# zilliztech/knowhere

Measured on NVIDIA H100. Metric: queries/sec at recall@10>=0.95, 10Mx128 f32 IVF_PQ, higher is better.
Workload: dtype f32

## Files before the change

### knowhere_b200/csrc/kb2_ivfpq_tc.cuh

```cuda
#pragma once
#include <cuda_bf16.h>

#include <type_traits>
#include <utility>

#include "kb2_gemm_tc.cuh"
#include "kb2_ivf.cuh"
#include "kb2_listmajor.cuh"

namespace kb2 {
namespace pqtc {

using lm::TM;
constexpr int NQT = 256;
constexpr int THREADS = 512;
constexpr int GROUP_THREADS = 128;
constexpr int MAXW = 80;
constexpr int META_BYTES = 3 * NQT * 4;
template <int G, int DSUB>
struct TcCfg {
    static constexpr int M = 16 * G;
    static constexpr int KD = M * DSUB;
    static_assert(KD % 16 == 0 && (DSUB == 2 || DSUB == 4 || DSUB == 8), "unsupported PQ geometry");
    static constexpr int XCHUNK = KD / 8;
    static constexpr int KSTEPS = KD / 16 + 1;
    static constexpr int CHUNKS = 2 * KSTEPS;
    static constexpr int GRP_BYTES = CHUNKS * 128;
    static constexpr int TAB_BYTES = M * 256 * DSUB * 2;
    static constexpr int A_BYTES = (TM / 8) * GRP_BYTES, B_BYTES = (NQT / 8) * GRP_BYTES;
    static constexpr int OFF_TAB = 0;
    static constexpr int OFF_A = TAB_BYTES;
    static constexpr int OFF_B = OFF_A + 2 * A_BYTES;
    static constexpr int OFF_META = OFF_B + B_BYTES;
    static constexpr int OFF_BAR = OFF_META + 2 * META_BYTES;
    static constexpr size_t SMEM_BYTES = OFF_BAR + 256 + 128 ;
    static_assert(SMEM_BYTES <= 227 * 1024, "filter kernel shared memory");
};
constexpr int KD = 128;
constexpr float kErrCoef = 0.0085f;
constexpr float kAccCoef = 4e-5f;

struct Params {
    int metric;
    int nq, nprobe;
    const float* queries;
    const __nv_bfloat16* qb16;
    const float* qnorm;
    const int32_t* n_items;
    int32_t* ticket;
    const int32_t* item_list;
    const int32_t* item_q0;
    const int32_t* item_nq;
    const int32_t* pair_q;
    const float* pair_base;
    const float* bound;
    int k_need;
    float margin_coef;
    float rmax;
    const int64_t* list_off;
    const int32_t* list_len;
    const uint4* codes;
    const uint4* codes_plain;
    int64_t npad;
    const float* t1;
    const float* pqc;
    const uint4* pqc16;
    const uint8_t* bitset;
    const int32_t* rows;
    uint4* log;
    uint32_t* log_cnt;
    uint32_t log_cap;
    uint32_t* qflag;
    unsigned long long* counters;
};

template <typename F, int... I>
__device__ __forceinline__ void
static_for_impl(F&& f, std::integer_sequence<int, I...>) {
    (f(std::integral_constant<int, I>{}), ...);
}
template <int N, typename F>
__device__ __forceinline__ void
static_for(F&& f) {
    static_for_impl(f, std::make_integer_sequence<int, N>{});
}
template <int C0_, int W_>
struct BlockCols {
    static constexpr int C0 = C0_, W = W_;
};
template <int LO, int HI, typename F>
__device__ __forceinline__ void
dispatch_range(int n, F&& f) {
    if constexpr (LO == HI) {
        f(std::integral_constant<int, LO>{});
    } else {
        constexpr int MID = (LO + HI) / 2;
        if (n <= MID) dispatch_range<LO, MID>(n, f);
        else dispatch_range<MID + 1, HI>(n, f);
    }
}

__device__ __forceinline__ void
bar_sync_epi() {
    asm volatile("bar.sync 1, 256;" ::: "memory");
}
__device__ __forceinline__ uint64_t
make_desc_ns(uint32_t smem_addr, uint32_t grp_bytes) {
    uint64_t d = 0;
    d |= (uint64_t)((smem_addr & 0x3FFFFu) >> 4);
    d |= (uint64_t)(128 >> 4) << 16;
    d |= (uint64_t)(grp_bytes >> 4) << 32;
    return d;
}

#ifdef KB2_FILTER_STALLS
#define KB2_STALL_BEGIN(v) const long long v = clock64()
#define KB2_STALL_END(slot, v) stall[slot] += clock64() - (v)
constexpr int kStallMaxCtas = 1024, kStallSlots = 8;
__device__ unsigned long long g_filter_stalls[kStallMaxCtas][2][2][kStallSlots];
__global__ void
filter_stalls_print_kernel(int ctas) {
    for (int b = 0; b < min(ctas, kStallMaxCtas); b++) {
        printf("KB2STALL cta=%d", b);
        for (int r = 0; r < 2; r++) {
            printf(r == 0 ? " dec=" : " cons=");
            for (int i = 0; i < kStallSlots; i++)
                printf(i ? ",%llu" : "%llu", g_filter_stalls[b][r][0][i] + g_filter_stalls[b][r][1][i]);
        }
        printf("\n");
    }
}
#else
#define KB2_STALL_BEGIN(v)
#define KB2_STALL_END(slot, v)
#endif

__device__ __forceinline__ void
split3_bf16(float x, uint32_t& hi, uint32_t& mid, uint32_t& lo) {
    const __nv_bfloat16 h = __float2bfloat16_rn(x);
    hi = (uint32_t)__bfloat16_as_ushort(h);
    if (!(fabsf(x) < INFINITY)) { mid = 0u; lo = 0u; return; }
    const float r1 = x - __bfloat162float(h);
    const __nv_bfloat16 m = __float2bfloat16_rn(r1);
    const float r2 = r1 - __bfloat162float(m);
    mid = (uint32_t)__bfloat16_as_ushort(m);
    lo = (uint32_t)__bfloat16_as_ushort(__float2bfloat16_rn(r2));
}

template <int METRIC, int G, int DSUB>
__global__ void __launch_bounds__(THREADS, 1)
ivfpq_tc_filter_kernel(Params p) {
    using C = TcCfg<G, DSUB>;
    constexpr int KD = C::KD, XCHUNK = C::XCHUNK, KSTEPS = C::KSTEPS, GRP_BYTES = C::GRP_BYTES, TAB_BYTES = C::TAB_BYTES;
    constexpr int A_BYTES = C::A_BYTES, OFF_TAB = C::OFF_TAB, OFF_A = C::OFF_A, OFF_B = C::OFF_B, OFF_META = C::OFF_META,
                  OFF_BAR = C::OFF_BAR;
    extern __shared__ unsigned char smem_dyn[];
    const uint32_t raw = tc::smem_u32(smem_dyn);
    const uint32_t base = (raw + 127u) & ~127u;
    unsigned char* sm = smem_dyn + (base - raw);
    const uint32_t bars = base + OFF_BAR;
    auto bar_a_full = [&](int i) { return bars + 8u * i; };
    auto bar_a_empty = [&](int i) { return bars + 8u * (2 + i); };
    const uint32_t bar_b_full = bars + 8u * 8, bar_b_free = bars + 8u * 9;
    auto bar_meta_full = [&](int i) { return bars + 8u * (10 + i); };
    auto bar_meta_free = [&](int i) { return bars + 8u * (12 + i); };
    uint32_t* qcnt = (uint32_t*)(sm + OFF_BAR + 8 * 15);

    const int warp = __shfl_sync(0xffffffffu, (int)threadIdx.x >> 5, 0), lane = threadIdx.x & 31;
    const int n_items = *p.n_items;

    const lm::ItemRing<8> ring(sm + OFF_BAR + 144, p.ticket);
    ring.init();

    if (threadIdx.x == 0) {
        for (int i = 0; i < 2; i++) {
            tc::mbar_init(bar_a_full(i), GROUP_THREADS);
            tc::mbar_init(bar_a_empty(i), GROUP_THREADS);
            tc::mbar_init(bar_meta_full(i), 2 * GROUP_THREADS);
            tc::mbar_init(bar_meta_free(i), 2 * GROUP_THREADS);
        }
        tc::mbar_init(bar_b_full, 2 * GROUP_THREADS);
        tc::mbar_init(bar_b_free, 2 * GROUP_THREADS);
        qcnt[0] = qcnt[1] = qcnt[2] = qcnt[3] = 0;
        asm volatile("fence.mbarrier_init.release.cluster;" ::: "memory");
    }
#ifdef KB2_FILTER_STALLS
    long long stall[kStallSlots] = {0, 0, 0, 0, 0, 0, 0, 0};
    KB2_STALL_BEGIN(t_role);
#endif
    {
        uint4* tab = (uint4*)(sm + OFF_TAB);
        for (int i = threadIdx.x; i < TAB_BYTES / 16; i += THREADS) tab[i] = __ldg(p.pqc16 + i);
    }
    __syncthreads();
    const float inv_alpha = (METRIC == KB2_METRIC_L2) ? 0.5f : 1.f;

    if (warp < 8) {
        const int dt = threadIdx.x;
        const int dg = dt >> 7;
        const int tid = dt & 127;
        const uint4* tab = (const uint4*)(sm + OFF_TAB);
        auto write_meta = [&](int item, int it) {
            KB2_STALL_BEGIN(t_meta);
            const int par = it & 1;
            tc::mbar_wait(bar_meta_free(par), (((uint32_t)it >> 1) & 1u) ^ 1u);
            const int q0 = p.item_q0[item];
            const int nqi = p.item_nq[item];
            float* m_h = (float*)(sm + OFF_META + par * META_BYTES);
            float* m_base = m_h + NQT;
            int* m_q = (int*)(m_base + NQT);
            const int j = dt;
            float h = -INFINITY, bs = 0.f;
            int q = -1;
            if (j < nqi) {
                q = p.pair_q[q0 + j];
                bs = p.pair_base[q0 + j];
                const float bnd = p.bound[q];
                if (!(bnd < INFINITY)) {
                    p.qflag[q] = 1u;
                    if (p.counters) atomicAdd(p.counters + 6, 1ull << 32);
                } else {
                    const float margin = p.margin_coef * p.qnorm[q] * 1.01f + 1e-30f;
                    const float h0 = (bnd + margin - bs) * inv_alpha;
                    h = h0 + kAccCoef * (fabsf(h0) + p.rmax) + 1e-30f;
                }
            }
            m_h[j] = h;
            m_base[j] = bs;
            m_q[j] = q;
            tc::mbar_arrive(bar_meta_full(par));
            KB2_STALL_END(5, t_meta);
        };
        uint32_t g0 = 0;
        int it = 0;
        int item = ring.at_warp(0);
        if (item < n_items) write_meta(item, 0);
        for (; item < n_items; it++) {
            const int item_next = ring.at_warp(it + 1);
            const int l = p.item_list[item];
            const int nqi = p.item_nq[item];
            const int nmma = (nqi + 15) & ~15;
            const int len = p.list_len[l];
            const int64_t off = p.list_off[l];
            const int ntiles = (len + TM - 1) / TM;
            const int par = it & 1;
            const int t_first = (int)((dg - (int)(g0 & 1u)) & 1);
            uint4 w_next[G];
#pragma unroll
            for (int g = 0; g < G; g++) w_next[g] = make_uint4(0, 0, 0, 0);
            float t_next = 0.f;
            const uint4* code_src = (DSUB == 8) ? p.codes : p.codes_plain;
            if (t_first < ntiles && off + (int64_t)t_first * TM + tid < p.npad) {
#pragma unroll
                for (int g = 0; g < G; g++) w_next[g] = ldg_stream_u4(code_src + (int64_t)g * p.npad + off + (int64_t)t_first * TM + tid);
                if (METRIC == KB2_METRIC_L2) t_next = __ldg(p.t1 + off + (int64_t)t_first * TM + tid);
            }
            auto decode_tile = [&](int t) {
                KB2_STALL_BEGIN(t_dec);
                const uint32_t g = g0 + (uint32_t)t;
                uint4 w[G];
#pragma unroll
                for (int gg = 0; gg < G; gg++) w[gg] = w_next[gg];
                const float tv = t_next;
                {
                    const int64_t pn = off + (int64_t)(t + 2) * TM + tid;
                    if (t + 2 < ntiles && pn < p.npad) {
#pragma unroll
                        for (int gg = 0; gg < G; gg++) w_next[gg] = ldg_stream_u4(code_src + (int64_t)gg * p.npad + pn);
                        if (METRIC == KB2_METRIC_L2) t_next = __ldg(p.t1 + pn);
                    }
                }
                float r = INFINITY;
                if (t * TM + tid < len) r = (METRIC == KB2_METRIC_L2) ? 0.5f * tv : 0.f;
                uint32_t rh, rm, rl;
                split3_bf16(-r, rh, rm, rl);
                uint4 v[XCHUNK];
                if constexpr (DSUB == 8) {
#pragma unroll
                    for (int gg = 0; gg < G; gg++) {
                        const uint32_t ww[4] = {w[gg].x, w[gg].y, w[gg].z, w[gg].w};
#pragma unroll
                        for (int s = 0; s < 16; s++) {
                            const uint32_t byte = (ww[s >> 2] >> (8 * (s & 3))) & 255u;
                            v[gg * 16 + s] = tab[byte * (16 * G) + gg * 16 + ((s + tid) & 15)];
                        }
                    }
                } else {
                    constexpr int SPC = 8 / DSUB;
                    constexpr int WPS = DSUB / 2;
                    const uint32_t* tab32 = reinterpret_cast<const uint32_t*>(tab);
#pragma unroll
                    for (int c = 0; c < XCHUNK; c++) {
                        uint32_t u[4];
#pragma unroll
                        for (int j = 0; j < SPC; j++) {
                            const int m = c * SPC + j;
                            const uint4 wg = w[m >> 4];
                            const int b = m & 15;
                            const uint32_t word = (b < 4) ? wg.x : (b < 8) ? wg.y : (b < 12) ? wg.z : wg.w;
                            const uint32_t byte = (word >> (8 * (b & 3))) & 255u;
#pragma unroll
                            for (int x = 0; x < WPS; x++) u[j * WPS + x] = tab32[(m * 256 + byte) * WPS + x];
                        }
                        v[c] = make_uint4(u[0], u[1], u[2], u[3]);
                    }
                }
                KB2_STALL_BEGIN(t_ae);
                tc::mbar_wait(bar_a_empty(dg), ((g >> 1) & 1u) ^ 1u);
                KB2_STALL_END(1, t_ae);
                unsigned char* A = sm + OFF_A + dg * A_BYTES + (tid >> 3) * GRP_BYTES + (tid & 7) * 16;
#pragma unroll
                for (int c = 0; c < XCHUNK; c++) {
                    const int chunk = (DSUB == 8) ? (c & ~15) + ((c + tid) & 15) : c;
                    *reinterpret_cast<uint4*>(A + chunk * 128) = v[c];
                }
                *reinterpret_cast<uint4*>(A + XCHUNK * 128) = make_uint4(rh | (rm << 16), rl | (0x3F80u << 16), 0x3F803F80u, 0u);
                *reinterpret_cast<uint4*>(A + (XCHUNK + 1) * 128) = make_uint4(0u, 0u, 0u, 0u);
                tc::fence_proxy_async();
                tc::mbar_arrive(bar_a_full(dg));
                KB2_STALL_END(3, t_dec);
            };
            if (t_first < ntiles) decode_tile(t_first);
            KB2_STALL_BEGIN(t_b);
            asm volatile("bar.sync 2, 256;" ::: "memory");
            KB2_STALL_BEGIN(t_bf);
            tc::mbar_wait(bar_b_free, ((uint32_t)it & 1u) ^ 1u);
            KB2_STALL_END(2, t_bf);
            {
                const float* m_h = (const float*)(sm + OFF_META + par * META_BYTES);
                const int* m_q = (const int*)(m_h + 2 * NQT);
                const uint32_t Bs = base + OFF_B;
                unsigned char* B = sm + OFF_B;
                const int kc = tid >> 3;
                const int rsub = tid & 7;
                for (int blk = dg; blk < nmma / 8 && kc < XCHUNK; blk += 2) {
                    const int row = blk * 8 + rsub;
                    const int q = m_q[row];
                    const uint32_t dst = (uint32_t)(blk * GRP_BYTES + kc * 128 + rsub * 16);
                    if (q >= 0) {
                        const void* src = reinterpret_cast<const uint4*>(p.qb16 + (int64_t)q * KD) + kc;
                        asm volatile("cp.async.cg.shared.global [%0], [%1], 16;" ::"r"(Bs + dst), "l"(src) : "memory");
                    } else {
                        *reinterpret_cast<uint4*>(B + dst) = make_uint4(0, 0, 0, 0);
                    }
                }
                if (dt < nmma) {
                    uint32_t hh, hm, hl;
                    split3_bf16(m_h[dt], hh, hm, hl);
                    unsigned char* Bc = B + (dt >> 3) * GRP_BYTES + (dt & 7) * 16;
                    *reinterpret_cast<uint4*>(Bc + XCHUNK * 128) = make_uint4(0x3F803F80u, 0x3F80u | (hh << 16), hm | (hl << 16), 0u);
                    *reinterpret_cast<uint4*>(Bc + (XCHUNK + 1) * 128) = make_uint4(0u, 0u, 0u, 0u);
                }
                asm volatile("cp.async.wait_all;" ::: "memory");
            }
            tc::fence_proxy_async();
            tc::mbar_arrive(bar_b_full);
            KB2_STALL_END(4, t_b);
            if (item_next < n_items) write_meta(item_next, it + 1);
            for (int t = t_first + 2; t < ntiles; t += 2) decode_tile(t);
            g0 += (uint32_t)ntiles;
            item = item_next;
        }
    } else {
        const int et = threadIdx.x - 256;
        const int eg = et >> 7;
        const int e = et & 127;
        const int we = warp & 3;
        const uint32_t n_logs = 2u * gridDim.x;
        uint4* my_log = p.log + (size_t)(2 * blockIdx.x + eg) * p.log_cap;
        uint32_t* my_cursor = qcnt + eg;
        bool log_over = false;
        unsigned long long n_codes = 0;
        uint32_t g0 = 0;
        int it = 0;
        for (int item = ring.at_warp(0); item < n_items; item = ring.at_warp(++it)) {
            const int l = p.item_list[item];
            const int nqi = p.item_nq[item];
            const int ncls = __shfl_sync(0xffffffffu, (nqi + 15) >> 4, 0);
            const int len = p.list_len[l];
            const int64_t off = p.list_off[l];
            const int ntiles = (len + TM - 1) / TM;
            const int par = it & 1;
            KB2_STALL_BEGIN(t_mf);
            tc::mbar_wait(bar_meta_full(par), ((uint32_t)it >> 1) & 1u);
            KB2_STALL_END(1, t_mf);
            const float* m_base = (const float*)(sm + OFF_META + par * META_BYTES) + NQT;
            const int* m_q = (const int*)(m_base + NQT);
            if (et == 0) n_codes += (unsigned long long)len * (unsigned long long)nqi;
            const int t_first = (int)((eg - (int)(g0 & 1u)) & 1);
            KB2_STALL_BEGIN(t_bfull);
            tc::mbar_wait(bar_b_full, (uint32_t)it & 1u);
            KB2_STALL_END(2, t_bfull);
            const uint32_t a0 = base + OFF_A + eg * A_BYTES;
            const uint32_t b0 = base + OFF_B;
            const uint32_t la0 = (uint32_t)make_desc_ns(a0, GRP_BYTES), lb0 = (uint32_t)make_desc_ns(b0, GRP_BYTES);
            constexpr uint64_t desc_hi = (uint64_t)(GRP_BYTES >> 4) << 32;
            for (int t = t_first; t < ntiles; t += 2) {
                const uint32_t g = g0 + (uint32_t)t;
                KB2_STALL_BEGIN(t_af);
                tc::mbar_wait(bar_a_full(eg), (g >> 1) & 1u);
                KB2_STALL_END(3, t_af);
                auto issue = [&](auto& acc, int h, auto blk) {
                    using B = decltype(blk);
                    KB2_STALL_BEGIN(t_is);
                    uint32_t la = la0 + (uint32_t)(h * 8 * GRP_BYTES / 16), lb = lb0 + (uint32_t)(B::C0 / 8 * GRP_BYTES / 16);
                    if constexpr (G == 1) asm volatile("" : "+r"(la), "+r"(lb));
                    tc::fence_operand(acc);
                    tc::wgmma_fence();
#pragma unroll
                    for (int ks = 0; ks < KSTEPS; ks++)
                        tc::wgmma_bf16<B::W>(acc, desc_hi | (la + ks * 16u), desc_hi | (lb + ks * 16u), ks > 0 ? 1u : 0u);
                    tc::wgmma_commit();
                    tc::fence_operand(acc);
                    KB2_STALL_END(6, t_is);
                };
                uint64_t mh[2][2] = {{0ull, 0ull}, {0ull, 0ull}};
                auto test = [&](const auto& v, int h, auto blk) {
                    using B = decltype(blk);
                    constexpr int NBIT = B::W / 4, HALF = NBIT / 2;
                    KB2_STALL_BEGIN(t_te);
                    uint32_t n0l = 0u, n0h = 0u, n1l = 0u, n1h = 0u;
#pragma unroll
                    for (int i = HALF - 1; i >= 0; i--) {
                        const int x = 4 * (i >> 1) + (i & 1);
                        const int xh = 4 * ((i + HALF) >> 1) + ((i + HALF) & 1);
                        n0l = __funnelshift_l(__float_as_uint(v[x]), n0l, 1);
                        n0h = __funnelshift_l(__float_as_uint(v[xh]), n0h, 1);
                        n1l = __funnelshift_l(__float_as_uint(v[x + 2]), n1l, 1);
                        n1h = __funnelshift_l(__float_as_uint(v[xh + 2]), n1h, 1);
                    }
                    constexpr uint32_t mask = (1u << NBIT) - 1u;
                    const uint32_t m0 = ~((n0h << HALF) | n0l) & mask, m1 = ~((n1h << HALF) | n1l) & mask;
                    mh[h][0] |= (uint64_t)m0 << (B::C0 / 4);
                    mh[h][1] |= (uint64_t)m1 << (B::C0 / 4);
                    KB2_STALL_END(7, t_te);
                };
                auto flush = [&]() {
                    const uint32_t total =
                        (uint32_t)(__popcll(mh[0][0]) + __popcll(mh[0][1]) + __popcll(mh[1][0]) + __popcll(mh[1][1]));
                    if (total != 0u) {
                        uint32_t slot = atomicAdd(my_cursor, total);
#pragma unroll
                        for (int h = 0; h < 2; h++) {
#pragma unroll
                            for (int i = 0; i < 2; i++) {
                                const int rel = t * TM + h * 64 + we * 16 + (lane >> 2) + 8 * i;
                                uint64_t m = mh[h][i];
                                while (m) {
                                    const int bit = __ffsll((long long)m) - 1;
                                    m &= m - 1;
                                    const int col = 8 * (bit >> 1) + 2 * (lane & 3) + (bit & 1);
                                    if (slot < p.log_cap) {
                                        uint4 o;
                                        o.x = (uint32_t)m_q[col];
                                        o.y = (uint32_t)(off + rel);
                                        o.z = __float_as_uint(m_base[col]);
                                        o.w = 0u;
                                        my_log[slot] = o;
                                    } else {
                                        log_over = true;
                                    }
                                    slot++;
                                }
                            }
                        }
                    }
                };
                dispatch_range<1, NQT / 16>(ncls, [&](auto nc) {
                    constexpr int NC = decltype(nc)::value, NB = (16 * NC + MAXW - 1) / MAXW, NBT = 2 * NB;
                    constexpr int U = NC / NB, X = NC % NB;
                    auto blk = [](auto cc) {
                        constexpr int c = decltype(cc)::value;
                        return BlockCols<16 * (c * U + (c < X ? c : X)), 16 * (U + (c < X ? 1 : 0))>{};
                    };
                    float va[8 * (U + (X > 0 ? 1 : 0))], vb[8 * (U + (X > 0 ? 1 : 0))];
                    issue(va, 0, blk(std::integral_constant<int, 0>{}));
                    static_for<NBT>([&](auto bc) {
                        constexpr int b = decltype(bc)::value;
                        if constexpr (b + 1 < NBT) {
                            constexpr auto bn = blk(std::integral_constant<int, (b + 1) % NB>{});
                            if constexpr ((b + 1) & 1) issue(vb, (b + 1) / NB, bn);
                            else issue(va, (b + 1) / NB, bn);
                            KB2_STALL_BEGIN(t_w);
                            tc::wgmma_wait<1>();
                            KB2_STALL_END(4, t_w);
                        } else {
                            KB2_STALL_BEGIN(t_w);
                            tc::wgmma_wait<0>();
                            KB2_STALL_END(4, t_w);
                        }
                        constexpr auto bb = blk(std::integral_constant<int, b % NB>{});
                        if constexpr (b & 1) {
                            tc::fence_operand(vb);
                            test(vb, b / NB, bb);
                        } else {
                            tc::fence_operand(va);
                            test(va, b / NB, bb);
                        }
                    });
                });
                tc::mbar_arrive(bar_a_empty(eg));
                KB2_STALL_BEGIN(t_fl);
                flush();
                KB2_STALL_END(5, t_fl);
            }
            tc::mbar_arrive(bar_b_free);
            tc::mbar_arrive(bar_meta_free(par));
            g0 += (uint32_t)ntiles;
        }
        if (log_over) p.log_cnt[n_logs] = 1u;
        if (eg == 0) asm volatile("bar.sync 3, 128;" ::: "memory"); else asm volatile("bar.sync 4, 128;" ::: "memory");
        if (e == 0) {
            const uint32_t n = min(*my_cursor, p.log_cap);
            p.log_cnt[2 * blockIdx.x + eg] = n;
            if (p.counters) atomicAdd(p.counters + 2, (unsigned long long)n);
        }
        if (et == 0 && p.counters) atomicAdd(p.counters, n_codes);
    }
#ifdef KB2_FILTER_STALLS
    KB2_STALL_END(0, t_role);
    if ((threadIdx.x & 127) == 0 && blockIdx.x < kStallMaxCtas) {
        for (int i = 0; i < kStallSlots; i++)
            g_filter_stalls[blockIdx.x][warp >= 8][(threadIdx.x >> 7) & 1][i] = (unsigned long long)stall[i];
    }
#endif
}

__global__ void
prepare_queries_kernel(const float* __restrict__ q, int64_t nq, int d, __nv_bfloat16* __restrict__ qb16, float* __restrict__ qnorm) {
    const int64_t w = ((int64_t)blockIdx.x * blockDim.x + threadIdx.x) >> 5;
    const int lane = threadIdx.x & 31;
    if (w >= nq) return;
    float s = 0.f;
    for (int j = lane * 4; j < d; j += 128) {
        const float4 v = __ldg(reinterpret_cast<const float4*>(q + w * d + j));
        __nv_bfloat162 lo = __floats2bfloat162_rn(v.x, v.y), hi = __floats2bfloat162_rn(v.z, v.w);
        uint2 o;
        o.x = *reinterpret_cast<uint32_t*>(&lo);
        o.y = *reinterpret_cast<uint32_t*>(&hi);
        *reinterpret_cast<uint2*>(qb16 + w * d + j) = o;
        s += v.x * v.x + v.y * v.y + v.z * v.z + v.w * v.w;
    }
    s = warp_sum(s);
    if (lane == 0) qnorm[w] = sqrtf(s) * 1.0001f;
}

__global__ void __launch_bounds__(256)
prepare_tables_kernel(const float* __restrict__ pqc, int dsub, __nv_bfloat16* __restrict__ pqc16, float* __restrict__ maxn2) {
    const int m = blockIdx.x, j = threadIdx.x;
    const int M = gridDim.x;
    const float* c = pqc + ((size_t)m * 256 + j) * dsub;
    float n2 = 0.f;
    __nv_bfloat16* o = pqc16 + (dsub == 8 ? ((size_t)j * M + m) : ((size_t)m * 256 + j)) * dsub;
    for (int t = 0; t < dsub; t++) {
        n2 = fmaf(c[t], c[t], n2);
        o[t] = __float2bfloat16_rn(c[t]);
    }
    __shared__ float red[256];
    red[j] = n2;
    __syncthreads();
    for (int s = 128; s > 0; s >>= 1) {
        if (j < s) red[j] = fmaxf(red[j], red[j + s]);
        __syncthreads();
    }
    if (j == 0) maxn2[m] = red[0];
}
__global__ void
unrotate_codes_kernel(const uint8_t* __restrict__ rot, int64_t total_words , int64_t npad, uint8_t* __restrict__ plain) {
    const int64_t t = (int64_t)blockIdx.x * blockDim.x + threadIdx.x;
    if (t >= total_words * 16) return;
    const int s = (int)(t & 15);
    const int64_t word = t >> 4;
    const int64_t pos = word % npad;
    plain[word * 16 + ((s + (int)(pos & 15)) & 15)] = rot[t];
}

template <int METRIC>
__global__ void __launch_bounds__(256, 1)
lut_build_kernel(const float* __restrict__ queries, int64_t nq, const int32_t* __restrict__ qlist, const uint32_t* __restrict__ qcount,
                 const float* __restrict__ pqc, float* __restrict__ lut) {
    __shared__ __align__(16) float s_q[2][KD];
    const int j = threadIdx.x;
    const float scale = (METRIC == KB2_METRIC_L2) ? -2.f : -1.f;
    if (qlist) nq = (int64_t)*qcount;
    float4 c[32];
#pragma unroll
    for (int m = 0; m < 16; m++) {
        const float* cp = pqc + ((size_t)m * 256 + j) * 8;
        c[2 * m] = __ldg(reinterpret_cast<const float4*>(cp));
        c[2 * m + 1] = __ldg(reinterpret_cast<const float4*>(cp + 4));
    }
    const int64_t per = (nq + gridDim.x - 1) / gridDim.x;
    const int64_t q_beg = (int64_t)blockIdx.x * per, q_end = min(nq, q_beg + per);
    auto qrow = [&](int64_t i) { return queries + (qlist ? (int64_t)qlist[i] : i) * KD; };
    if (q_beg < q_end && threadIdx.x < KD) s_q[0][threadIdx.x] = qrow(q_beg)[threadIdx.x];
    __syncthreads();
    for (int64_t q = q_beg; q < q_end; q++) {
        const int cur = (int)((q - q_beg) & 1);
        if (q + 1 < q_end && threadIdx.x < KD) s_q[cur ^ 1][threadIdx.x] = qrow(q + 1)[threadIdx.x];
        float* dst = lut + q * 4096 + j * 16;
#pragma unroll
        for (int m4 = 0; m4 < 16; m4 += 4) {
            float o[4];
#pragma unroll
            for (int u = 0; u < 4; u++) {
                const int m = m4 + u;
                const float4 qa = *reinterpret_cast<const float4*>(&s_q[cur][m * 8]);
                const float4 qb = *reinterpret_cast<const float4*>(&s_q[cur][m * 8 + 4]);
                float a = 0.f;
                a = fmaf(qa.x, c[2 * m].x, a); a = fmaf(qa.y, c[2 * m].y, a); a = fmaf(qa.z, c[2 * m].z, a); a = fmaf(qa.w, c[2 * m].w, a);
                a = fmaf(qb.x, c[2 * m + 1].x, a); a = fmaf(qb.y, c[2 * m + 1].y, a); a = fmaf(qb.z, c[2 * m + 1].z, a); a = fmaf(qb.w, c[2 * m + 1].w, a);
                o[u] = a * scale;
            }
            *reinterpret_cast<float4*>(dst + m4) = make_float4(o[0], o[1], o[2], o[3]);
        }
        __syncthreads();
    }
}

template <int METRIC, int G, int DSUB>
__global__ void __launch_bounds__(128)
exact_eval_kernel(const float* __restrict__ queries, const float* __restrict__ pqc, const float* __restrict__ lut,
                  const float* __restrict__ bound_of,
                  const uint4* __restrict__ codes, int64_t npad, const float* __restrict__ t1, const uint8_t* __restrict__ bitset,
                  const int32_t* __restrict__ rows, uint64_t* __restrict__ cand, uint32_t* __restrict__ cand_cnt, int cap,
                  uint32_t* __restrict__ qflag, const uint32_t* __restrict__ log_over, int k_trim = 0) {
    constexpr int KDIM = 16 * G * DSUB;
    __shared__ __align__(16) float s_q[KDIM];
    __shared__ uint32_t s_h[256];
    __shared__ float s_red[8];
    __shared__ uint32_t s_ctl[2];
    const int64_t q = blockIdx.x;
    if (*log_over) {
        if (threadIdx.x == 0) qflag[q] = 1u;
        return;
    }
    if (qflag[q]) return;
    const uint32_t n = min(cand_cnt[q], (uint32_t)cap);
    if (n == 0) return;
    const bool use_lut = (G == 1 && DSUB == 8) && lut != nullptr;
    if (!use_lut) {
        for (int j = threadIdx.x; j < KDIM; j += 128) s_q[j] = queries[q * KDIM + j];
        __syncthreads();
    }
    const float* lq = lut + q * 4096;
    const float bound = bound_of[q];
    const float scale = (METRIC == KB2_METRIC_L2) ? -2.f : -1.f;
    uint64_t* row = cand + q * cap;
    auto eval = [&](uint64_t ent, float& key_out) -> uint64_t {
        const uint32_t pos = (uint32_t)ent;
        const float base = __uint_as_float((uint32_t)(ent >> 32));
        float acc0 = (METRIC == KB2_METRIC_L2) ? __ldg(t1 + pos) : 0.f, acc1 = 0.f;
#pragma unroll
        for (int g = 0; g < G; g++) {
            const uint4 w = __ldg(codes + (int64_t)g * npad + pos);
            const uint32_t ww[4] = {w.x, w.y, w.z, w.w};
#pragma unroll
            for (int s = 0; s < 16; s++) {
                const uint32_t byte = (ww[s >> 2] >> (8 * (s & 3))) & 255u;
                const uint32_t m = g * 16 + ((pos + s) & 15u);
                float v;
                if (use_lut) {
                    v = __ldg(lq + byte * 16 + m);
                } else {
                    const float* c = pqc + ((size_t)m * 256 + byte) * DSUB;
                    const float* qs = &s_q[m * DSUB];
                    float a = 0.f;
#pragma unroll
                    for (int t = 0; t < DSUB; t++) a = fmaf(qs[t], __ldg(c + t), a);
                    v = __fmul_rn(a, scale);
                }
                if (s & 1) acc1 = __fadd_rn(acc1, v); else acc0 = __fadd_rn(acc0, v);
            }
        }
        const float key = __fadd_rn(base, __fadd_rn(acc0, acc1));
        bool keep = key <= bound;
        if (keep && bitset) keep = !bit_is_set(bitset, rows[pos]);
        key_out = keep ? key : INFINITY;
        return keep ? pack_kp(key, pos) : kEmpty;
    };
    if (k_trim > 0 && n <= 512u && n > (uint32_t)k_trim) {
        uint64_t pk[4];
        float kf[4];
        float lo = INFINITY, hi = -INFINITY;
        s_h[threadIdx.x] = 0;
        s_h[threadIdx.x + 128] = 0;
        if (threadIdx.x == 0) s_ctl[1] = 0;
#pragma unroll
        for (int it = 0; it < 4; it++) {
            const uint32_t i = threadIdx.x + it * 128;
            pk[it] = kEmpty;
            kf[it] = INFINITY;
            if (i < n) pk[it] = eval(row[i], kf[it]);
            if (kf[it] < INFINITY) { lo = fminf(lo, kf[it]); hi = fmaxf(hi, kf[it]); }
        }
#pragma unroll
        for (int o = 16; o > 0; o >>= 1) {
            lo = fminf(lo, __shfl_xor_sync(0xffffffffu, lo, o));
            hi = fmaxf(hi, __shfl_xor_sync(0xffffffffu, hi, o));
        }
        if ((threadIdx.x & 31) == 0) { s_red[threadIdx.x >> 5] = lo; s_red[4 + (threadIdx.x >> 5)] = hi; }
        __syncthreads();
        lo = fminf(fminf(s_red[0], s_red[1]), fminf(s_red[2], s_red[3]));
        hi = fmaxf(fmaxf(s_red[4], s_red[5]), fmaxf(s_red[6], s_red[7]));
        const float sc = (hi > lo) ? 256.f / (hi - lo) : 0.f;
        int bin[4];
#pragma unroll
        for (int it = 0; it < 4; it++) {
            bin[it] = 256;
            if (kf[it] < INFINITY) {
                bin[it] = min(255, (int)((kf[it] - lo) * sc));
                atomicAdd(&s_h[bin[it]], 1u);
            }
        }
        __syncthreads();
        if (threadIdx.x < 32) {
            const int lane = threadIdx.x;
            uint32_t h[8], sum = 0;
#pragma unroll
            for (int t = 0; t < 8; t++) { h[t] = s_h[lane * 8 + t]; sum += h[t]; }
            uint32_t incl = sum;
#pragma unroll
            for (int o = 1; o < 32; o <<= 1) {
                const uint32_t v = __shfl_up_sync(0xffffffffu, incl, o);
                if (lane >= o) incl += v;
            }
            const uint32_t excl = incl - sum;
            const uint32_t total = __shfl_sync(0xffffffffu, incl, 31);
            if (lane == 0 && total < (uint32_t)k_trim) s_ctl[0] = 255u;
            if (excl < (uint32_t)k_trim && incl >= (uint32_t)k_trim) {
                uint32_t run = excl;
                int b = lane * 8 + 7;
#pragma unroll
                for (int t = 0; t < 8; t++) {
                    run += h[t];
                    if (run >= (uint32_t)k_trim) { b = lane * 8 + t; break; }
                }
                s_ctl[0] = (uint32_t)b;
            }
        }
        __syncthreads();
        const int bstar = (int)s_ctl[0];
#pragma unroll
        for (int it = 0; it < 4; it++)
            if (bin[it] <= bstar) row[atomicAdd(&s_ctl[1], 1u)] = pk[it];
        __syncthreads();
        if (threadIdx.x == 0) cand_cnt[q] = s_ctl[1];
        return;
    }
    float lo = INFINITY, hi = -INFINITY;
    for (uint32_t i = threadIdx.x; i < n; i += 128) {
        float kf;
        row[i] = eval(row[i], kf);
        if (kf < INFINITY) { lo = fminf(lo, kf); hi = fmaxf(hi, kf); }
    }
    if (k_trim > 0 && k_trim <= 96 && n > 512u) {
        __shared__ uint64_t s_stage[128];
        s_h[threadIdx.x] = 0;
        s_h[threadIdx.x + 128] = 0;
        if (threadIdx.x == 0) { s_ctl[0] = 0xffffffffu; s_ctl[1] = 0; }
#pragma unroll
        for (int o = 16; o > 0; o >>= 1) {
            lo = fminf(lo, __shfl_xor_sync(0xffffffffu, lo, o));
            hi = fmaxf(hi, __shfl_xor_sync(0xffffffffu, hi, o));
        }
        if ((threadIdx.x & 31) == 0) { s_red[threadIdx.x >> 5] = lo; s_red[4 + (threadIdx.x >> 5)] = hi; }
        __syncthreads();
        lo = fminf(fminf(s_red[0], s_red[1]), fminf(s_red[2], s_red[3]));
        hi = fmaxf(fmaxf(s_red[4], s_red[5]), fmaxf(s_red[6], s_red[7]));
        const float sc = (hi > lo) ? 256.f / (hi - lo) : 0.f;
        for (uint32_t i = threadIdx.x; i < n; i += 128) {
            const uint64_t e = row[i];
            if (e != kEmpty) atomicAdd(&s_h[min(255, (int)((unpack_key(e) - lo) * sc))], 1u);
        }
        __syncthreads();
        if (threadIdx.x < 32) {
            const int lane = threadIdx.x;
            uint32_t h[8], sum = 0;
#pragma unroll
            for (int t = 0; t < 8; t++) { h[t] = s_h[lane * 8 + t]; sum += h[t]; }
            uint32_t incl = sum;
#pragma unroll
            for (int o = 1; o < 32; o <<= 1) {
                const uint32_t v = __shfl_up_sync(0xffffffffu, incl, o);
                if (lane >= o) incl += v;
            }
            const uint32_t excl = incl - sum;
            if (excl < (uint32_t)k_trim && incl >= (uint32_t)k_trim) {
                uint32_t run = excl;
                int b = lane * 8 + 7;
#pragma unroll
                for (int t = 0; t < 8; t++) {
                    run += h[t];
                    if (run >= (uint32_t)k_trim) { b = lane * 8 + t; break; }
                }
                if (run <= 128u) s_ctl[0] = (uint32_t)b;
            }
        }
        __syncthreads();
        const uint32_t bstar = s_ctl[0];
        if (bstar == 0xffffffffu) return;
        for (uint32_t i = threadIdx.x; i < n; i += 128) {
            const uint64_t e = row[i];
            if (e != kEmpty && (uint32_t)min(255, (int)((unpack_key(e) - lo) * sc)) <= bstar) s_stage[atomicAdd(&s_ctl[1], 1u)] = e;
        }
        __syncthreads();
        const uint32_t nk = s_ctl[1];
        for (uint32_t i = threadIdx.x; i < nk; i += 128) row[i] = s_stage[i];
        if (threadIdx.x == 0) cand_cnt[q] = nk;
    }
}

__global__ void __launch_bounds__(1024)
compact_resp_kernel(const int64_t* __restrict__ probe_ids, int nprobe, int64_t nq, const int32_t* __restrict__ list_owner, int rank,
                    int32_t* __restrict__ list, uint32_t* __restrict__ count) {
    __shared__ uint32_t s_n;
    if (threadIdx.x == 0) s_n = 0;
    __syncthreads();
    for (int64_t q = threadIdx.x; q < nq; q += 1024) {
        const int64_t l = probe_ids[q * nprobe];
        if (l >= 0 && list_owner[l] == rank) list[atomicAdd(&s_n, 1u)] = (int32_t)q;
    }
    __syncthreads();
    if (threadIdx.x == 0) *count = s_n;
}
__global__ void
fill_f32_kernel(float* __restrict__ out, int64_t n, float v) {
    const int64_t i = (int64_t)blockIdx.x * blockDim.x + threadIdx.x;
    if (i < n) out[i] = v;
}
__global__ void __launch_bounds__(256)
max_abs_kernel(const float* __restrict__ x, int64_t n, uint32_t* __restrict__ out) {
    float m = 0.f;
    for (int64_t i = (int64_t)blockIdx.x * blockDim.x + threadIdx.x; i < n; i += (int64_t)gridDim.x * blockDim.x) m = fmaxf(m, fabsf(x[i]));
#pragma unroll
    for (int o = 16; o > 0; o >>= 1) m = fmaxf(m, __shfl_xor_sync(0xffffffffu, m, o));
    if ((threadIdx.x & 31) == 0 && m > 0.f) atomicMax(out, __float_as_uint(m));
}

__global__ void __launch_bounds__(1024)
compact_flags_kernel(const uint32_t* __restrict__ qflag, int64_t nq, int32_t* __restrict__ list, uint32_t* __restrict__ count) {
    __shared__ uint32_t s_n;
    if (threadIdx.x == 0) s_n = 0;
    __syncthreads();
    for (int64_t q = threadIdx.x; q < nq; q += 1024)
        if (qflag[q]) list[atomicAdd(&s_n, 1u)] = (int32_t)q;
    __syncthreads();
    if (threadIdx.x == 0) *count = s_n;
}

#define KB2_BOUND_STEP(WORD, KB, S, ACC)                                                      \
    {                                                                                         \
        const uint32_t _x = __byte_perm((WORD), lane4, 0x6504u | ((KB) << 4));                \
        float _v;                                                                             \
        asm("ld.shared.f32 %0, [%1+%2];" : "=f"(_v) : "r"(_x >> 1), "n"(KB2_SMEM_BASE + 4 * (S))); \
        ACC += _v;                                                                            \
    }
__global__ void
transpose_codebook_kernel(const float* __restrict__ pqc, int M, int dsub, float* __restrict__ pqc_t) {
    const int64_t i = (int64_t)blockIdx.x * blockDim.x + threadIdx.x;
    const int64_t n = (int64_t)M * 256 * dsub;
    if (i >= n) return;
    const int x = (int)(i % dsub);
    const int j = (int)((i / dsub) % 256);
    const int m = (int)(i / ((int64_t)dsub * 256));
    pqc_t[((((int64_t)(m >> 4) * 256 + j) * 16) + (m & 15)) * dsub + x] = pqc[i];
}
constexpr int BOUND_KMAX = 6144;
constexpr int BOUND_BINS = 1024;
__host__ __device__ constexpr int bound_kmax(int min_codes, int k_need) {
    const int want = ((min_codes > k_need ? min_codes : k_need) + 63) & ~63;
    return want < BOUND_KMAX ? want : BOUND_KMAX;
}
constexpr size_t bound_smem(int kmax) { return (size_t)32 * 1024 + (size_t)kmax * 4 + BOUND_BINS * 4 + 128; }

template <int METRIC, int G, int DSUB, int NT>
__global__ void __launch_bounds__(NT)
bound_kernel(const float* __restrict__ lut, const int32_t* __restrict__ qlist, const uint32_t* __restrict__ qcount, int64_t nq,
             const int64_t* __restrict__ probe_ids, const float* __restrict__ probe_dis,
             int probe_stride, int p0_max, int min_codes, int k_need, const int64_t* __restrict__ list_off,
             const int32_t* __restrict__ list_len, const uint4* __restrict__ codes, const float* __restrict__ t1,
             const uint8_t* __restrict__ bitset, const int32_t* __restrict__ rows, float* __restrict__ out,
             unsigned long long* __restrict__ counters, int64_t npad = 0, const float* __restrict__ queries = nullptr,
             const float* __restrict__ pqc_t = nullptr) {
    static_assert(NT == 128 || NT == 256, "bound_kernel block size");
    constexpr int NW = NT / 32;
    constexpr int BPT = BOUND_BINS / NT;
    extern __shared__ __align__(16) unsigned char smem_raw[];
    float* s_lut = (float*)smem_raw;
    const int key_cap = bound_kmax(min_codes, k_need);
    float* s_keys = (float*)(smem_raw + 32 * 1024);
    uint32_t* s_hist = (uint32_t*)(s_keys + key_cap);
    float* s_red = (float*)(s_hist + BOUND_BINS);
    const int warp = threadIdx.x >> 5, lane = threadIdx.x & 31;
    if ((uint32_t)__cvta_generic_to_shared(smem_raw) != (uint32_t)KB2_SMEM_BASE) {
        if (threadIdx.x == 0 && counters) atomicExch(counters + 1, 0xBAD5ull);
        return;
    }
    const int64_t n_work = qlist ? (int64_t)*qcount : nq;
    for (int64_t wi = blockIdx.x; wi < n_work; wi += gridDim.x) {
    const int64_t q = qlist ? (int64_t)qlist[wi] : wi;
    int seen = 0, n_tot = 0;
    float kmin = INFINITY, kmax = -INFINITY;
#pragma unroll 1
    for (int g = 0; g < G; g++) {
    __syncthreads();
    if constexpr (G > 1 || DSUB != 8) {
        const float scale = (METRIC == KB2_METRIC_L2) ? -2.f : -1.f;
        const int mm = threadIdx.x & 15, jsub = threadIdx.x >> 4;
        float qv[DSUB];
#pragma unroll
        for (int x = 0; x < DSUB; x++) qv[x] = queries[q * (int64_t)(16 * G * DSUB) + (g * 16 + mm) * DSUB + x];
        for (int j = jsub; j < 256; j += NT / 16) {
            const float* cp = pqc_t + (((size_t)g * 256 + j) * 16 + mm) * DSUB;
            float a = 0.f;
#pragma unroll
            for (int x = 0; x < DSUB; x++) a = fmaf(qv[x], __ldg(cp + x), a);
            a *= scale;
            s_lut[j * 32 + mm] = a;
            s_lut[j * 32 + 16 + mm] = a;
        }
    } else {
        const float4* src = reinterpret_cast<const float4*>(lut + wi * 4096);
#pragma unroll
        for (int i = 0; i < 1024 / NT; i++) {
            const int idx = threadIdx.x + i * NT;
            const float4 v = __ldg(src + idx);
            float4* dst = reinterpret_cast<float4*>(s_lut + (idx >> 2) * 32 + (idx & 3) * 4);
            dst[0] = v;
            dst[4] = v;
        }
    }
    if (g == 0)
        for (int i = threadIdx.x; i < BOUND_BINS; i += NT) s_hist[i] = 0;
    __syncthreads();
    const uint32_t lane4 = (uint32_t)(lane & 15) << 3;
    const uint4* gcodes = codes + (int64_t)g * npad;
    const bool first_g = (g == 0), last_g = (g == G - 1);
    seen = 0;
    n_tot = 0;
    const int code_cap = min(key_cap, max(min_codes, k_need));
    for (int j = 0; j < p0_max && seen < min_codes && n_tot < code_cap; j++) {
        const int64_t l = probe_ids[q * probe_stride + j];
        if (l < 0) continue;
        const int len_all = list_len[l];
        if (len_all == 0) continue;
        seen += len_all;
        const int len = min(len_all, code_cap - n_tot);
        const int64_t off = list_off[l];
        const float dv = probe_dis[q * probe_stride + j];
        const float base = (METRIC == KB2_METRIC_L2) ? dv : -dv;
        uint4 nA = make_uint4(0, 0, 0, 0), nB = nA;
        float ntA = 0.f, ntB = 0.f;
        auto load_iter = [&](int c0) {
            if (c0 < len) {
                nA = ldg_stream_u4(gcodes + off + c0 + lane);
                if (METRIC == KB2_METRIC_L2 && first_g) ntA = __ldg(t1 + off + c0 + lane);
                if (c0 + 32 < len) {
                    nB = ldg_stream_u4(gcodes + off + c0 + 32 + lane);
                    if (METRIC == KB2_METRIC_L2 && first_g) ntB = __ldg(t1 + off + c0 + 32 + lane);
                }
            }
        };
        load_iter(warp * 64);
        for (int c0 = warp * 64; c0 < len; c0 += NW * 64) {
            const int relA = c0 + lane, relB = c0 + 32 + lane;
            const bool okA = relA < len, okB = relB < len;
            const uint32_t posA = (uint32_t)(off + relA), posB = (uint32_t)(off + relB);
            const bool hasB = c0 + 32 < len;
            const uint4 wA = nA;
            const uint4 wB = hasB ? nB : nA;
            float a0 = ntA, a1 = 0.f, b0 = hasB ? ntB : 0.f, b1 = 0.f;
            load_iter(c0 + NW * 64);
            KB2_BOUND_STEP(wA.x, 0, 0, a0)  KB2_BOUND_STEP(wB.x, 0, 0, b0)  KB2_BOUND_STEP(wA.x, 1, 1, a1)  KB2_BOUND_STEP(wB.x, 1, 1, b1)
            KB2_BOUND_STEP(wA.x, 2, 2, a0)  KB2_BOUND_STEP(wB.x, 2, 2, b0)  KB2_BOUND_STEP(wA.x, 3, 3, a1)  KB2_BOUND_STEP(wB.x, 3, 3, b1)
            KB2_BOUND_STEP(wA.y, 0, 4, a0)  KB2_BOUND_STEP(wB.y, 0, 4, b0)  KB2_BOUND_STEP(wA.y, 1, 5, a1)  KB2_BOUND_STEP(wB.y, 1, 5, b1)
            KB2_BOUND_STEP(wA.y, 2, 6, a0)  KB2_BOUND_STEP(wB.y, 2, 6, b0)  KB2_BOUND_STEP(wA.y, 3, 7, a1)  KB2_BOUND_STEP(wB.y, 3, 7, b1)
            KB2_BOUND_STEP(wA.z, 0, 8, a0)  KB2_BOUND_STEP(wB.z, 0, 8, b0)  KB2_BOUND_STEP(wA.z, 1, 9, a1)  KB2_BOUND_STEP(wB.z, 1, 9, b1)
            KB2_BOUND_STEP(wA.z, 2, 10, a0) KB2_BOUND_STEP(wB.z, 2, 10, b0) KB2_BOUND_STEP(wA.z, 3, 11, a1) KB2_BOUND_STEP(wB.z, 3, 11, b1)
            KB2_BOUND_STEP(wA.w, 0, 12, a0) KB2_BOUND_STEP(wB.w, 0, 12, b0) KB2_BOUND_STEP(wA.w, 1, 13, a1) KB2_BOUND_STEP(wB.w, 1, 13, b1)
            KB2_BOUND_STEP(wA.w, 2, 14, a0) KB2_BOUND_STEP(wB.w, 2, 14, b0) KB2_BOUND_STEP(wA.w, 3, 15, a1) KB2_BOUND_STEP(wB.w, 3, 15, b1)
            float keyA = (first_g ? base : s_keys[n_tot + (okA ? relA : 0)]) + (a0 + a1);
            float keyB = (first_g ? base : s_keys[n_tot + ((hasB && okB) ? relB : 0)]) + (b0 + b1);
            if (okA) {
                if (last_g && bitset && bit_is_set(bitset, rows[posA])) keyA = INFINITY;
                s_keys[n_tot + relA] = keyA;
                if (last_g && keyA < INFINITY) { kmin = fminf(kmin, keyA); kmax = fmaxf(kmax, keyA); }
            }
            if (hasB && okB) {
                if (last_g && bitset && bit_is_set(bitset, rows[posB])) keyB = INFINITY;
                s_keys[n_tot + relB] = keyB;
                if (last_g && keyB < INFINITY) { kmin = fminf(kmin, keyB); kmax = fmaxf(kmax, keyB); }
            }
        }
        n_tot += len;
    }
    }
#pragma unroll
    for (int o = 16; o > 0; o >>= 1) {
        kmin = fminf(kmin, __shfl_xor_sync(0xffffffffu, kmin, o));
        kmax = fmaxf(kmax, __shfl_xor_sync(0xffffffffu, kmax, o));
    }
    if (lane == 0) { s_red[warp] = kmin; s_red[8 + warp] = kmax; }
    __syncthreads();
    float lo = s_red[0], hi = s_red[8];
#pragma unroll
    for (int w = 1; w < NW; w++) { lo = fminf(lo, s_red[w]); hi = fmaxf(hi, s_red[8 + w]); }
    const float scale = (hi > lo) ? (float)BOUND_BINS / (hi - lo) : 0.f;
    for (int i = threadIdx.x; i < n_tot; i += NT) {
        const float kv = s_keys[i];
        if (kv < INFINITY) atomicAdd(&s_hist[min(BOUND_BINS - 1, (int)((kv - lo) * scale))], 1u);
    }
    __syncthreads();
    uint32_t mine[BPT], tsum = 0;
#pragma unroll
    for (int b = 0; b < BPT; b++) { mine[b] = s_hist[threadIdx.x * BPT + b]; tsum += mine[b]; }
    uint32_t incl = tsum;
#pragma unroll
    for (int o = 1; o < 32; o <<= 1) {
        const uint32_t v = __shfl_up_sync(0xffffffffu, incl, o);
        if (lane >= o) incl += v;
    }
    uint32_t* s_wsum = (uint32_t*)(s_red + 16);
    if (lane == 31) s_wsum[warp] = incl;
    __syncthreads();
    uint32_t before = incl - tsum;
    for (int w = 0; w < warp; w++) before += s_wsum[w];
    uint32_t total = 0;
#pragma unroll
    for (int w = 0; w < NW; w++) total += s_wsum[w];
    const uint32_t need = (uint32_t)k_need;
    if (total < need || seen < 4 * k_need) {
        if (threadIdx.x == 0) out[q] = INFINITY;
    } else if (before < need && before + tsum >= need) {
        uint32_t cum = before;
        int b = 0;
#pragma unroll
        for (int bb = 0; bb < BPT; bb++) {
            if (cum < need) { cum += mine[bb]; b = bb; }
        }
        const float bound = (scale > 0.f) ? lo + ((float)(threadIdx.x * BPT + b) + 1.01f) / scale : hi;
        out[q] = fmaxf(bound, lo) + (G == 1 ? 4e-7f : 2e-6f) * fmaxf(fabsf(lo), fabsf(hi));
    }
    }
}
#undef KB2_BOUND_STEP

}
}
```

Baseline: 4.290 million.

## Move candidate log expansion from MMA warps to decode warps via shared masks

New measurement: 4.266 million (median of 6 runs). About the same (-0.5%).

```diff
diff --git a/knowhere_b200/csrc/kb2_ivfpq_tc.cuh b/knowhere_b200/csrc/kb2_ivfpq_tc.cuh
--- a/knowhere_b200/csrc/kb2_ivfpq_tc.cuh
+++ b/knowhere_b200/csrc/kb2_ivfpq_tc.cuh
@@ -17,6 +17,7 @@
 constexpr int GROUP_THREADS = 128;
 constexpr int MAXW = 80;
 constexpr int META_BYTES = 3 * NQT * 4;
+constexpr int MASK_BYTES = 2 * GROUP_THREADS * 16;
 template <int G, int DSUB>
 struct TcCfg {
     static constexpr int M = 16 * G;
@@ -32,7 +33,8 @@
     static constexpr int OFF_A = TAB_BYTES;
     static constexpr int OFF_B = OFF_A + 2 * A_BYTES;
     static constexpr int OFF_META = OFF_B + B_BYTES;
-    static constexpr int OFF_BAR = OFF_META + 2 * META_BYTES;
+    static constexpr int OFF_MASK = OFF_META + 2 * META_BYTES;
+    static constexpr int OFF_BAR = OFF_MASK + 2 * MASK_BYTES;
     static constexpr size_t SMEM_BYTES = OFF_BAR + 256 + 128 ;
     static_assert(SMEM_BYTES <= 227 * 1024, "filter kernel shared memory");
 };
@@ -153,7 +155,7 @@
     using C = TcCfg<G, DSUB>;
     constexpr int KD = C::KD, XCHUNK = C::XCHUNK, KSTEPS = C::KSTEPS, GRP_BYTES = C::GRP_BYTES, TAB_BYTES = C::TAB_BYTES;
     constexpr int A_BYTES = C::A_BYTES, OFF_TAB = C::OFF_TAB, OFF_A = C::OFF_A, OFF_B = C::OFF_B, OFF_META = C::OFF_META,
-                  OFF_BAR = C::OFF_BAR;
+                  OFF_MASK = C::OFF_MASK, OFF_BAR = C::OFF_BAR;
     extern __shared__ unsigned char smem_dyn[];
     const uint32_t raw = tc::smem_u32(smem_dyn);
     const uint32_t base = (raw + 127u) & ~127u;
@@ -162,7 +164,6 @@
     auto bar_a_full = [&](int i) { return bars + 8u * i; };
     auto bar_a_empty = [&](int i) { return bars + 8u * (2 + i); };
     const uint32_t bar_b_full = bars + 8u * 8, bar_b_free = bars + 8u * 9;
-    auto bar_meta_full = [&](int i) { return bars + 8u * (10 + i); };
     auto bar_meta_free = [&](int i) { return bars + 8u * (12 + i); };
     uint32_t* qcnt = (uint32_t*)(sm + OFF_BAR + 8 * 15);
 
@@ -176,12 +177,11 @@
         for (int i = 0; i < 2; i++) {
             tc::mbar_init(bar_a_full(i), GROUP_THREADS);
             tc::mbar_init(bar_a_empty(i), GROUP_THREADS);
-            tc::mbar_init(bar_meta_full(i), 2 * GROUP_THREADS);
             tc::mbar_init(bar_meta_free(i), 2 * GROUP_THREADS);
         }
         tc::mbar_init(bar_b_full, 2 * GROUP_THREADS);
         tc::mbar_init(bar_b_free, 2 * GROUP_THREADS);
-        qcnt[0] = qcnt[1] = qcnt[2] = qcnt[3] = 0;
+        qcnt[0] = qcnt[1] = 0;
         asm volatile("fence.mbarrier_init.release.cluster;" ::: "memory");
     }
 #ifdef KB2_FILTER_STALLS
@@ -228,8 +228,62 @@
             m_h[j] = h;
             m_base[j] = bs;
             m_q[j] = q;
-            tc::mbar_arrive(bar_meta_full(par));
             KB2_STALL_END(5, t_meta);
+        };
+        bool pend = false;
+        uint32_t pend_g = 0, pend_pos = 0;
+        int pend_par = 0;
+        auto take_masks = [&](uint4& ma, uint4& mb) {
+            const uint4* my_masks = (const uint4*)(sm + OFF_MASK + dg * MASK_BYTES) + tid;
+            ma = my_masks[0];
+            mb = my_masks[GROUP_THREADS];
+        };
+        auto expand = [&](const uint4& ma, const uint4& mb) {
+            KB2_STALL_BEGIN(t_ex);
+            const uint64_t mh[2][2] = {{ma.x | ((uint64_t)ma.y << 32), ma.z | ((uint64_t)ma.w << 32)},
+                                       {mb.x | ((uint64_t)mb.y << 32), mb.z | ((uint64_t)mb.w << 32)}};
+            const uint32_t total = (uint32_t)(__popcll(mh[0][0]) + __popcll(mh[0][1]) + __popcll(mh[1][0]) + __popcll(mh[1][1]));
+            if (total != 0u) {
+                const float* m_base = (const float*)(sm + OFF_META + pend_par * META_BYTES) + NQT;
+                const int* m_q = (const int*)(m_base + NQT);
+                uint4* my_log = p.log + (size_t)(2 * blockIdx.x + dg) * p.log_cap;
+                uint32_t slot = atomicAdd(qcnt + dg, total);
+#pragma unroll
+                for (int h = 0; h < 2; h++) {
+#pragma unroll
+                    for (int i = 0; i < 2; i++) {
+                        const uint32_t pos = pend_pos + (uint32_t)(h * 64 + (tid >> 5) * 16 + (lane >> 2) + 8 * i);
+                        uint64_t m = mh[h][i];
+                        while (m) {
+                            const int bit = __ffsll((long long)m) - 1;
+                            m &= m - 1;
+                            const int col = 8 * (bit >> 1) + 2 * (lane & 3) + (bit & 1);
+                            if (slot < p.log_cap) {
+                                uint4 o;
+                                o.x = (uint32_t)m_q[col];
+                                o.y = pos;
+                                o.z = __float_as_uint(m_base[col]);
+                                o.w = 0u;
+                                my_log[slot] = o;
+                            } else {
+                                p.log_cnt[2u * gridDim.x] = 1u;
+                            }
+                            slot++;
+                        }
+                    }
+                }
+            }
+            KB2_STALL_END(7, t_ex);
+        };
+        auto drain = [&]() {
+            if (!pend) return;
+            KB2_STALL_BEGIN(t_pk);
+            tc::mbar_wait(bar_a_empty(dg), (pend_g >> 1) & 1u);
+            uint4 ma, mb;
+            take_masks(ma, mb);
+            KB2_STALL_END(6, t_pk);
+            expand(ma, mb);
+            pend = false;
         };
         uint32_t g0 = 0;
         int it = 0;
@@ -308,6 +362,10 @@
                 KB2_STALL_BEGIN(t_ae);
                 tc::mbar_wait(bar_a_empty(dg), ((g >> 1) & 1u) ^ 1u);
                 KB2_STALL_END(1, t_ae);
+                KB2_STALL_END(3, t_dec);
+                KB2_STALL_BEGIN(t_pk);
+                KB2_STALL_END(6, t_pk);
+                KB2_STALL_BEGIN(t_st);
                 unsigned char* A = sm + OFF_A + dg * A_BYTES + (tid >> 3) * GRP_BYTES + (tid & 7) * 16;
 #pragma unroll
                 for (int c = 0; c < XCHUNK; c++) {
@@ -317,8 +375,15 @@
                 *reinterpret_cast<uint4*>(A + XCHUNK * 128) = make_uint4(rh | (rm << 16), rl | (0x3F80u << 16), 0x3F803F80u, 0u);
                 *reinterpret_cast<uint4*>(A + (XCHUNK + 1) * 128) = make_uint4(0u, 0u, 0u, 0u);
                 tc::fence_proxy_async();
+                uint4 ma, mb;
+                if (pend) take_masks(ma, mb);
                 tc::mbar_arrive(bar_a_full(dg));
-                KB2_STALL_END(3, t_dec);
+                KB2_STALL_END(3, t_st);
+                if (pend) expand(ma, mb);
+                pend = true;
+                pend_g = g;
+                pend_pos = (uint32_t)(off + (int64_t)t * TM);
+                pend_par = par;
             };
             if (t_first < ntiles) decode_tile(t_first);
             KB2_STALL_BEGIN(t_b);
@@ -356,20 +421,28 @@
             tc::fence_proxy_async();
             tc::mbar_arrive(bar_b_full);
             KB2_STALL_END(4, t_b);
+            if (it > 0) {
+                if (pend_par != par) drain();
+                tc::mbar_arrive(bar_meta_free(par ^ 1));
+            }
             if (item_next < n_items) write_meta(item_next, it + 1);
             for (int t = t_first + 2; t < ntiles; t += 2) decode_tile(t);
             g0 += (uint32_t)ntiles;
             item = item_next;
         }
+        drain();
+        if (dg == 0) asm volatile("bar.sync 3, 128;" ::: "memory"); else asm volatile("bar.sync 4, 128;" ::: "memory");
+        if (tid == 0) {
+            const uint32_t n = min(qcnt[dg], p.log_cap);
+            p.log_cnt[2 * blockIdx.x + dg] = n;
+            if (p.counters) atomicAdd(p.counters + 2, (unsigned long long)n);
+        }
     } else {
         const int et = threadIdx.x - 256;
         const int eg = et >> 7;
         const int e = et & 127;
-        const int we = warp & 3;
-        const uint32_t n_logs = 2u * gridDim.x;
-        uint4* my_log = p.log + (size_t)(2 * blockIdx.x + eg) * p.log_cap;
-        uint32_t* my_cursor = qcnt + eg;
-        bool log_over = false;
+        const uint32_t my_masks_s = base + OFF_MASK + eg * MASK_BYTES + e * 16;
+        uint4* my_masks = (uint4*)(sm + OFF_MASK + eg * MASK_BYTES) + e;
         unsigned long long n_codes = 0;
         uint32_t g0 = 0;
         int it = 0;
@@ -378,14 +451,7 @@
             const int nqi = p.item_nq[item];
             const int ncls = __shfl_sync(0xffffffffu, (nqi + 15) >> 4, 0);
             const int len = p.list_len[l];
-            const int64_t off = p.list_off[l];
             const int ntiles = (len + TM - 1) / TM;
-            const int par = it & 1;
-            KB2_STALL_BEGIN(t_mf);
-            tc::mbar_wait(bar_meta_full(par), ((uint32_t)it >> 1) & 1u);
-            KB2_STALL_END(1, t_mf);
-            const float* m_base = (const float*)(sm + OFF_META + par * META_BYTES) + NQT;
-            const int* m_q = (const int*)(m_base + NQT);
             if (et == 0) n_codes += (unsigned long long)len * (unsigned long long)nqi;
             const int t_first = (int)((eg - (int)(g0 & 1u)) & 1);
             KB2_STALL_BEGIN(t_bfull);
@@ -404,7 +470,7 @@
                     using B = decltype(blk);
                     KB2_STALL_BEGIN(t_is);
                     uint32_t la = la0 + (uint32_t)(h * 8 * GRP_BYTES / 16), lb = lb0 + (uint32_t)(B::C0 / 8 * GRP_BYTES / 16);
-                    if constexpr (G == 1) asm volatile("" : "+r"(la), "+r"(lb));
+                    asm volatile("" : "+r"(la), "+r"(lb));
                     tc::fence_operand(acc);
                     tc::wgmma_fence();
 #pragma unroll
@@ -434,37 +500,6 @@
                     mh[h][0] |= (uint64_t)m0 << (B::C0 / 4);
                     mh[h][1] |= (uint64_t)m1 << (B::C0 / 4);
                     KB2_STALL_END(7, t_te);
-                };
-                auto flush = [&]() {
-                    const uint32_t total =
-                        (uint32_t)(__popcll(mh[0][0]) + __popcll(mh[0][1]) + __popcll(mh[1][0]) + __popcll(mh[1][1]));
-                    if (total != 0u) {
-                        uint32_t slot = atomicAdd(my_cursor, total);
-#pragma unroll
-                        for (int h = 0; h < 2; h++) {
-#pragma unroll
-                            for (int i = 0; i < 2; i++) {
-                                const int rel = t * TM + h * 64 + we * 16 + (lane >> 2) + 8 * i;
-                                uint64_t m = mh[h][i];
-                                while (m) {
-                                    const int bit = __ffsll((long long)m) - 1;
-                                    m &= m - 1;
-                                    const int col = 8 * (bit >> 1) + 2 * (lane & 3) + (bit & 1);
-                                    if (slot < p.log_cap) {
-                                        uint4 o;
-                                        o.x = (uint32_t)m_q[col];
-                                        o.y = (uint32_t)(off + rel);
-                                        o.z = __float_as_uint(m_base[col]);
-                                        o.w = 0u;
-                                        my_log[slot] = o;
-                                    } else {
-                                        log_over = true;
-                                    }
-                                    slot++;
-                                }
-                            }
-                        }
-                    }
                 };
                 dispatch_range<1, NQT / 16>(ncls, [&](auto nc) {
                     constexpr int NC = decltype(nc)::value, NB = (16 * NC + MAXW - 1) / MAXW, NBT = 2 * NB;
@@ -497,23 +532,18 @@
                             tc::fence_operand(va);
                             test(va, b / NB, bb);
                         }
+                        if constexpr (b == NB - 1)
+                            asm volatile("st.shared.v2.b64 [%0], {%1, %2};" ::"r"(my_masks_s), "l"(mh[0][0]), "l"(mh[0][1]) : "memory");
                     });
                 });
+                KB2_STALL_BEGIN(t_ms);
+                my_masks[GROUP_THREADS] =
+                    make_uint4((uint32_t)mh[1][0], (uint32_t)(mh[1][0] >> 32), (uint32_t)mh[1][1], (uint32_t)(mh[1][1] >> 32));
+                KB2_STALL_END(5, t_ms);
                 tc::mbar_arrive(bar_a_empty(eg));
-                KB2_STALL_BEGIN(t_fl);
-                flush();
-                KB2_STALL_END(5, t_fl);
             }
             tc::mbar_arrive(bar_b_free);
-            tc::mbar_arrive(bar_meta_free(par));
             g0 += (uint32_t)ntiles;
-        }
-        if (log_over) p.log_cnt[n_logs] = 1u;
-        if (eg == 0) asm volatile("bar.sync 3, 128;" ::: "memory"); else asm volatile("bar.sync 4, 128;" ::: "memory");
-        if (e == 0) {
-            const uint32_t n = min(*my_cursor, p.log_cap);
-            p.log_cnt[2 * blockIdx.x + eg] = n;
-            if (p.counters) atomicAdd(p.counters + 2, (unsigned long long)n);
         }
         if (et == 0 && p.counters) atomicAdd(p.counters, n_codes);
     }
```
